# iden3/wasmsnark

Measured on AMD Instinct MI355X. Metric: BN128 Groth16 prove ms @ 2^20 constraints, lower is better.
Workload: dtype u256 (Montgomery; 9x29-bit limbs, v_mad_u64_u32); 1 GPU; BN128 full Groth16 prove, synthetic 2^20-constraint R1CS (1-3 non-zeros per column of A and B, every variable present), key and witness resident in HBM, r and s injected; parallelism=1 GPU, no collective, lanes=2, device=AMD Radeon Graphics gfx950:sramecc+:xnack- CUs=256 device=0

## Files before the change

wasmsnark_amd/csrc/msm.hip:

```cpp
#include <string.h>

#include <algorithm>
#include <chrono>

#include "internal.h"
namespace wsnark {

#ifndef WS_ACC_WAVES
#define WS_ACC_WAVES 3
#endif
#ifndef WS_ACC_WAVES_G2
#define WS_ACC_WAVES_G2 2
#endif
#ifndef WS_G2_PREFETCH
#define WS_G2_PREFETCH 0
#endif
#ifndef WS_G1_PREFETCH
#define WS_G1_PREFETCH 1
#endif
#ifndef WS_MADD_WIDE
#define WS_MADD_WIDE 1
#endif
static const uint32_t CHUNK = 8;
#ifndef WS_TAIL_L2_DEFAULT
#define WS_TAIL_L2_DEFAULT 4
#endif

struct MsmScratch {
    DevBuf vals_out, entries, hot, hot_sums;
    DevBuf bstart, bend, buckets, counters, tasks, multi, partials;
    DevBuf chunkS, chunkA, sums, points_conv;
    DevBuf hot_done;
    DevBuf tree_half, tree_done;
};

static const uint32_t PRESORT_MAX_BINS = 4096;
static const uint32_t CNT_HIST = 16, CNT_CURSOR = 16 + 512, CNT_BINS = 2048;

template <class Fn>
__device__ __forceinline__ void for_each_digit(const Fe& raw, uint32_t c, uint32_t Wall, uint32_t w_off, uint32_t w_stride, Fn f) {
    const Fe s = Fr::reduce_full(raw);
    const uint32_t NB = 1u << (c - 1);
    uint32_t carry = 0, k = 0;
    for (uint32_t w = 0; w < Wall; w++) {
        const uint32_t bit = w * c;
        const uint32_t limb = bit >> 6, off = bit & 63;
        uint64_t v = limb < 4 ? (s.l[limb] >> off) : 0;
        if (off + c > 64 && limb + 1 < 4) v |= s.l[limb + 1] << (64 - off);
        uint32_t d = (uint32_t)(v & ((1u << c) - 1)) + carry;
        uint32_t neg = 0;
        if (d > NB) { d = (1u << c) - d; neg = 1; carry = 1; } else carry = 0;
        if (w >= w_off && (w - w_off) % w_stride == 0) {
            if (d) f(k, d, neg);
            k++;
        }
    }
}

struct PresortArgs {
    const Fe* scalars;
    uint32_t n, c, Wall, w_off, w_stride;
    uint32_t i0, i_end;
    uint32_t lo_bits, HB, nbins;
    uint32_t tile;
    uint32_t idx_bits;
    const uint8_t* mask;
    uint32_t flat;
};
__device__ __forceinline__ uint32_t presort_bin(const PresortArgs& A, uint32_t k, uint32_t d) {
    return (A.flat ? 0u : k * A.HB) + ((d - 1) >> A.lo_bits);
}

template <class E> struct PresortEntry;
template <> struct PresortEntry<uint64_t> {
    static __device__ __forceinline__ uint64_t make(uint32_t i, uint32_t neg, uint32_t lo, uint32_t) {
        return ((uint64_t)lo << 32) | (uint64_t)(i | (neg << 31));
    }
    static __device__ __forceinline__ uint32_t lo(uint64_t e, uint32_t) { return (uint32_t)(e >> 32); }
    static __device__ __forceinline__ uint32_t val(uint64_t e, uint32_t) { return (uint32_t)e; }
};
template <> struct PresortEntry<uint32_t> {
    static __device__ __forceinline__ uint32_t make(uint32_t i, uint32_t neg, uint32_t lo, uint32_t ib) {
        return i | (neg << ib) | (lo << (ib + 1));
    }
    static __device__ __forceinline__ uint32_t lo(uint32_t e, uint32_t ib) { return e >> (ib + 1); }
    static __device__ __forceinline__ uint32_t val(uint32_t e, uint32_t ib) {
        return (e & ((1u << ib) - 1)) | (((e >> ib) & 1u) << 31);
    }
};

__global__ __launch_bounds__(1024) void presort_count(PresortArgs A, uint32_t* __restrict__ bin_count) {
    __shared__ uint32_t cnt[PRESORT_MAX_BINS];
    for (uint32_t b = threadIdx.x; b < A.nbins; b += blockDim.x) cnt[b] = 0;
    __syncthreads();
    const uint32_t base = A.i0 + blockIdx.x * A.tile;
    for (uint32_t i = base + threadIdx.x; i < base + A.tile && i < A.i_end; i += blockDim.x) {
        if (A.mask && !A.mask[i]) continue;
        for_each_digit(A.scalars[i], A.c, A.Wall, A.w_off, A.w_stride, [&](uint32_t k, uint32_t d, uint32_t) {
            atomicAdd(&cnt[presort_bin(A, k, d)], 1u);
        });
    }
    __syncthreads();
    for (uint32_t b = threadIdx.x; b < A.nbins; b += blockDim.x)
        if (cnt[b]) atomicAdd(&bin_count[b], cnt[b]);
}

__global__ __launch_bounds__(256) void presort_scan(const uint32_t* __restrict__ bin_count, uint32_t nbins,
                                                      uint32_t* __restrict__ bin_start, uint32_t* __restrict__ bin_cursor) {
    __shared__ uint32_t part[256];
    const uint32_t per = (nbins + 255) / 256, lo = threadIdx.x * per;
    uint32_t sum = 0;
    for (uint32_t b = lo; b < lo + per && b < nbins; b++) sum += bin_count[b];
    part[threadIdx.x] = sum;
    __syncthreads();
    if (threadIdx.x == 0) {
        uint32_t run = 0;
        for (uint32_t t = 0; t < 256; t++) { const uint32_t v = part[t]; part[t] = run; run += v; }
        bin_start[nbins] = run;
    }
    __syncthreads();
    uint32_t run = part[threadIdx.x];
    for (uint32_t b = lo; b < lo + per && b < nbins; b++) {
        bin_start[b] = run;
        bin_cursor[b] = run;
        run += bin_count[b];
    }
}

template <class E>
__global__ __launch_bounds__(1024) void presort_scatter(PresortArgs A, uint32_t* __restrict__ bin_cursor, E* __restrict__ entries) {
    __shared__ uint32_t cnt[PRESORT_MAX_BINS];
    __shared__ uint32_t gbase[PRESORT_MAX_BINS];
    for (uint32_t b = threadIdx.x; b < A.nbins; b += blockDim.x) cnt[b] = 0;
    __syncthreads();
    const uint32_t base = A.i0 + blockIdx.x * A.tile;
    for (uint32_t i = base + threadIdx.x; i < base + A.tile && i < A.i_end; i += blockDim.x) {
        if (A.mask && !A.mask[i]) continue;
        for_each_digit(A.scalars[i], A.c, A.Wall, A.w_off, A.w_stride, [&](uint32_t k, uint32_t d, uint32_t) {
            atomicAdd(&cnt[presort_bin(A, k, d)], 1u);
        });
    }
    __syncthreads();
    for (uint32_t b = threadIdx.x; b < A.nbins; b += blockDim.x) {
        const uint32_t c0 = cnt[b];
        gbase[b] = c0 ? atomicAdd(&bin_cursor[b], c0) : 0;
        cnt[b] = 0;
    }
    __syncthreads();
    const uint32_t lo_mask = (1u << A.lo_bits) - 1;
    for (uint32_t i = base + threadIdx.x; i < base + A.tile && i < A.i_end; i += blockDim.x) {
        if (A.mask && !A.mask[i]) continue;
        for_each_digit(A.scalars[i], A.c, A.Wall, A.w_off, A.w_stride, [&](uint32_t k, uint32_t d, uint32_t neg) {
            const uint32_t b = presort_bin(A, k, d);
            const uint32_t r = atomicAdd(&cnt[b], 1u);
            const uint32_t idx = A.flat ? (A.w_off + k * A.w_stride) * A.n + i : i;
            entries[gbase[b] + r] = PresortEntry<E>::make(idx, neg, (d - 1) & lo_mask, A.idx_bits);
        });
    }
}

static const uint32_t PRESORT_ONCE_W = 16;
__device__ __forceinline__ uint32_t block_exclusive_scan(uint32_t v, uint32_t* wsum, uint32_t* total) {
    const uint32_t lane = threadIdx.x & 63, wid = threadIdx.x >> 6, nw = (blockDim.x + 63) >> 6;
    uint32_t x = v;
    for (uint32_t d = 1; d < 64; d <<= 1) {
        const uint32_t y = __shfl(x, (int)(lane >= d ? lane - d : lane));
        if (lane >= d) x += y;
    }
    if (lane == 63) wsum[wid] = x;
    __syncthreads();
    if (wid == 0) {
        const uint32_t w = lane < nw ? wsum[lane] : 0;
        uint32_t t = w;
        for (uint32_t d = 1; d < 64; d <<= 1) {
            const uint32_t y = __shfl(t, (int)(lane >= d ? lane - d : lane));
            if (lane >= d) t += y;
        }
        if (lane < nw) wsum[lane] = t - w;
        if (lane == 63) wsum[16] = t;
    }
    __syncthreads();
    *total = wsum[16];
    return wsum[wid] + x - v;
}
template <class E>
__global__ __launch_bounds__(1024) void presort_scatter_once(PresortArgs A, const uint32_t* __restrict__ bin_count,
                                                               uint32_t* __restrict__ bin_start, uint32_t* __restrict__ bin_cursor,
                                                               E* __restrict__ entries) {
    __shared__ uint32_t cnt[PRESORT_MAX_BINS];
    __shared__ uint32_t gbase[PRESORT_MAX_BINS];
    __shared__ uint32_t wsum[17];
    {
        const uint32_t per = (A.nbins + blockDim.x - 1) / blockDim.x, b0 = threadIdx.x * per;
        uint32_t mine = 0, total;
        for (uint32_t b = b0; b < b0 + per && b < A.nbins; b++) mine += bin_count[b];
        uint32_t run = block_exclusive_scan(mine, wsum, &total);
        for (uint32_t b = b0; b < b0 + per && b < A.nbins; b++) {
            gbase[b] = run;
            if (blockIdx.x == 0) bin_start[b] = run;
            run += bin_count[b];
            cnt[b] = 0;
        }
        if (blockIdx.x == 0 && threadIdx.x == 0) bin_start[A.nbins] = total;
    }
    __syncthreads();
    const uint32_t i = A.i0 + blockIdx.x * blockDim.x + threadIdx.x;
    const bool live = i < A.i_end && (!A.mask || A.mask[i]);
    const uint32_t NONE = 0xFFFFFFFFu;
    E ent[PRESORT_ONCE_W];
    uint32_t where[PRESORT_ONCE_W];
    {
        const Fe s = live ? Fr::reduce_full(A.scalars[i]) : Fe{{0, 0, 0, 0}};
        const uint32_t c = A.c, NB = 1u << (c - 1), lo_mask = (1u << A.lo_bits) - 1;
        uint32_t carry = 0, k = 0, next_own = A.w_off;
#pragma unroll
        for (uint32_t w = 0; w < PRESORT_ONCE_W; w++) {
            where[w] = NONE;
            ent[w] = 0;
            if (w < A.Wall) {
                const uint32_t bit = w * c, limb = bit >> 6, off = bit & 63;
                const uint64_t lo = limb == 0 ? s.l[0] : limb == 1 ? s.l[1] : limb == 2 ? s.l[2] : limb == 3 ? s.l[3] : 0;
                const uint64_t hi = limb == 0 ? s.l[1] : limb == 1 ? s.l[2] : limb == 2 ? s.l[3] : 0;
                uint64_t v = lo >> off;
                if (off + c > 64) v |= hi << (64 - off);
                uint32_t d = (uint32_t)(v & ((1u << c) - 1)) + carry;
                uint32_t neg = 0;
                if (d > NB) { d = (1u << c) - d; neg = 1; carry = 1; } else carry = 0;
                if (w == next_own) {
                    if (live && d) {
                        const uint32_t b = presort_bin(A, k, d);
                        where[w] = b | (atomicAdd(&cnt[b], 1u) << 12);
                        ent[w] = PresortEntry<E>::make(A.flat ? w * A.n + i : i, neg, (d - 1) & lo_mask, A.idx_bits);
                    }
                    k++;
                    next_own += A.w_stride;
                }
            }
        }
    }
    __syncthreads();
    for (uint32_t b = threadIdx.x; b < A.nbins; b += blockDim.x) {
        const uint32_t c0 = cnt[b];
        if (c0) gbase[b] += atomicAdd(&bin_cursor[b], c0);
    }
    __syncthreads();
#pragma unroll
    for (uint32_t w = 0; w < PRESORT_ONCE_W; w++)
        if (where[w] != NONE) entries[gbase[where[w] & 0xFFFu] + (where[w] >> 12)] = ent[w];
}

__device__ __forceinline__ uint32_t len_key(uint32_t len, uint32_t lmax) {
    uint32_t k = (len * 255u + lmax - 1) / lmax;
    return k > 255u ? 255u : (k < 1u ? 1u : k);
}

static const uint32_t PRESORT_MAX_LO = 10;
__device__ __forceinline__ uint32_t wave_rank_add(uint32_t* counters, uint32_t key, bool active) {
    const unsigned long long act = __ballot(active);
    if (act == 0) return 0;
    const uint32_t lane = threadIdx.x & 63;
    const int first = __ffsll(act) - 1;
    const uint32_t k0 = __shfl(key, first);
    const unsigned long long same = __ballot(active && key == k0);
    uint32_t r = 0;
    if (same == act) {
        uint32_t base = 0;
        if (lane == (uint32_t)first) base = atomicAdd(&counters[k0], (uint32_t)__popcll(act));
        base = __shfl(base, first);
        r = base + (uint32_t)__popcll(act & ((1ull << lane) - 1));
    } else if (active) {
        r = atomicAdd(&counters[key], 1u);
    }
    return r;
}

template <class E>
__global__ __launch_bounds__(1024) void presort_bins(const E* __restrict__ entries, const uint32_t* __restrict__ bin_start,
                                                       uint32_t lo_bits, uint32_t idx_bits, uint32_t* __restrict__ vals_out,
                                                       uint32_t* __restrict__ bstart, uint32_t* __restrict__ bend,
                                                       uint32_t lmax, uint32_t* __restrict__ hist,
                                                       const uint8_t* __restrict__ mask, uint32_t mask_mod) {
    __shared__ uint32_t sub[1u << PRESORT_MAX_LO];
    __shared__ uint32_t off[1u << PRESORT_MAX_LO];
    __shared__ uint32_t wsum[17];
    __shared__ uint32_t lhist[256];
    const uint32_t bin = blockIdx.x, SUB = 1u << lo_bits;
    const uint32_t s = bin_start[bin], e = bin_start[bin + 1];
    for (uint32_t t = threadIdx.x; t < SUB; t += blockDim.x) sub[t] = 0;
    for (uint32_t t = threadIdx.x; t < 256; t += blockDim.x) lhist[t] = 0;
    __syncthreads();
    const uint32_t stride = 4 * blockDim.x;
    const uint32_t iters = (e - s + stride - 1) / stride;
    for (uint32_t it = 0; it < iters; it++) {
        const uint32_t i = s + threadIdx.x + it * stride;
        E v[4];
#pragma unroll
        for (uint32_t u = 0; u < 4; u++) {
            const uint32_t j = i + u * blockDim.x;
            v[u] = j < e ? entries[j] : (E)0;
        }
#pragma unroll
        for (uint32_t u = 0; u < 4; u++) {
            bool active = i + u * blockDim.x < e;
            if (mask && active) {
                const uint32_t idx = PresortEntry<E>::val(v[u], idx_bits) & 0x7FFFFFFFu;
                active = mask[mask_mod ? idx % mask_mod : idx] != 0;
            }
            (void)wave_rank_add(sub, PresortEntry<E>::lo(v[u], idx_bits), active);
        }
    }
    __syncthreads();
    const uint32_t per = (SUB + blockDim.x - 1) / blockDim.x, t0 = threadIdx.x * per;
    uint32_t mine = 0, bin_total;
    for (uint32_t t = t0; t < t0 + per && t < SUB; t++) mine += sub[t];
    uint32_t run = s + block_exclusive_scan(mine, wsum, &bin_total);
    for (uint32_t t = t0; t < t0 + per && t < SUB; t++) {
        const uint32_t cnt = sub[t];
        const uint32_t bucket = (bin << lo_bits) + t;
        off[t] = run;
        bstart[bucket] = run;
        bend[bucket] = run + cnt;
        run += cnt;
        sub[t] = 0;
        if (cnt) {
            const uint32_t nt = (cnt + lmax - 1) / lmax, rem = cnt - (nt - 1) * lmax;
            if (nt > 1) atomicAdd(&lhist[255], nt - 1);
            atomicAdd(&lhist[len_key(rem, lmax)], 1u);
        }
    }
    __syncthreads();
    for (uint32_t t = threadIdx.x; t < 256; t += blockDim.x)
        if (lhist[t]) atomicAdd(&hist[t], lhist[t]);
    for (uint32_t it = 0; it < iters; it++) {
        const uint32_t i = s + threadIdx.x + it * stride;
        E v[4];
#pragma unroll
        for (uint32_t u = 0; u < 4; u++) {
            const uint32_t j = i + u * blockDim.x;
            v[u] = j < e ? entries[j] : (E)0;
        }
#pragma unroll
        for (uint32_t u = 0; u < 4; u++) {
            bool active = i + u * blockDim.x < e;
            if (mask && active) {
                const uint32_t idx = PresortEntry<E>::val(v[u], idx_bits) & 0x7FFFFFFFu;
                active = mask[mask_mod ? idx % mask_mod : idx] != 0;
            }
            const uint32_t lo = PresortEntry<E>::lo(v[u], idx_bits);
            const uint32_t r = wave_rank_add(sub, lo, active);
            if (active) vals_out[off[lo] + r] = PresortEntry<E>::val(v[u], idx_bits);
        }
    }
}

#ifndef WS_ACC_FAST
#define WS_ACC_FAST 1
#endif
#ifndef WS_ACC_MMADD
#define WS_ACC_MMADD 1
#endif
template <class C>
__device__ __forceinline__ typename C::Pt accumulate_range(const typename C::AffP* __restrict__ points,
                                                           const uint32_t* __restrict__ vals, uint32_t s, uint32_t len) {
    typedef typename C::Field F;
    typename C::Pt acc = C::infinity();
    if (len == 0) return acc;
    constexpr bool kPrefetch = sizeof(typename C::AffP) > 64 ? WS_G2_PREFETCH != 0 : WS_G1_PREFETCH != 0;
    uint32_t k = 0;
#if WS_ACC_FAST && WS_MADD_WIDE
    {
        uint32_t v = vals[s];
        typename C::AffP cp = points[v & 0x7FFFFFFFu];
        if (!F::packed_is_zero(cp.x)) {
            typename C::Aff a0 = C::unpack_aff(cp);
            a0.y = F::cneg(a0.y, (v >> 31) != 0);
            acc = typename C::Pt{a0.x, a0.y, F::one(), F::one()};
            k = 1;
            const uint32_t last = len - 1;
#if WS_ACC_MMADD
            if (len > 1) {
                v = vals[s + 1];
                cp = points[v & 0x7FFFFFFFu];
                if (!F::packed_is_zero(cp.x) && C::mmadd_fast(acc, a0, C::unpack_aff(cp), (v >> 31) != 0)) k = 2;
            }
#endif
            if (kPrefetch) {
                uint32_t v1 = vals[s + (k < last ? k : last)], v2 = vals[s + (k + 1 < last ? k + 1 : last)];
                cp = points[v1 & 0x7FFFFFFFu];
                while (k < len) {
                    const bool inf = F::packed_is_zero(cp.x);
                    typename C::Aff cur = C::unpack_aff(cp);
                    const bool neg = (v1 >> 31) != 0;
                    F::keep(cur.x);
                    F::keep(cur.y);
                    v1 = v2;
                    cp = points[v1 & 0x7FFFFFFFu];
                    v2 = vals[s + (k + 2 < last ? k + 2 : last)];
                    if (inf) break;
                    if (!C::madd_fast(acc, cur, neg)) break;
                    k++;
                }
            } else {
                uint32_t vn = vals[s + (k < last ? k : last)];
                while (k < len) {
                    v = vn;
                    cp = points[v & 0x7FFFFFFFu];
                    vn = vals[s + (k + 1 < last ? k + 1 : last)];
                    if (F::packed_is_zero(cp.x)) break;
                    if (!C::madd_fast(acc, C::unpack_aff(cp), (v >> 31) != 0)) break;
                    k++;
                }
            }
        }
    }
#endif
    if (k < len) {
        if (!kPrefetch) {
            for (; k < len; k++) {
                const uint32_t v = vals[s + k];
                const typename C::Aff cur = C::unpack_aff(points[v & 0x7FFFFFFFu]);
#if WS_MADD_WIDE
                C::madd_wide(acc, cur, (v >> 31) != 0);
#else
                C::madd(acc, cur, (v >> 31) != 0);
#endif
            }
        } else {
            uint32_t v = vals[s + k];
            typename C::AffP nxt = points[v & 0x7FFFFFFFu];
            for (; k < len; k++) {
                const typename C::Aff cur = C::unpack_aff(nxt);
                const bool neg = (v >> 31) != 0;
                if (k + 1 < len) {
                    v = vals[s + k + 1];
                    nxt = points[v & 0x7FFFFFFFu];
                }
#if WS_MADD_WIDE
                C::madd_wide(acc, cur, neg);
#else
                C::madd(acc, cur, neg);
#endif
            }
        }
    }
    C::narrow_x(acc);
    return acc;
}

template <class C>
__global__ __launch_bounds__(256) void msm_convert_points(const typename C::AffP* __restrict__ in,
                                                            typename C::AffP* __restrict__ out, uint64_t n) {
    const uint64_t i = (uint64_t)blockIdx.x * blockDim.x + threadIdx.x;
    if (i >= n) return;
    out[i] = C::pack_aff(C::aff_to_internal(in[i]));
}

static const uint32_t PARTIAL_FLAG = 0x80000000u;
struct Task { uint32_t dst, start, len; };
struct MultiBucket { uint32_t bucket, first_partial, ntasks; };
static const uint32_t HOT_MIN = 1024;
static const uint32_t HOT_SLICE = 512;
struct HotBucket { uint32_t bucket, first_partial, ntasks, task_base, rem_index, start, rem, slice_base; };

__global__ __launch_bounds__(256) void msm_plan_emit(const uint32_t* __restrict__ bstart, const uint32_t* __restrict__ bend,
                                                       uint32_t nbuckets, uint32_t lmax, const uint32_t* __restrict__ hist,
                                                       uint32_t* __restrict__ cursor,
                                                       Task* __restrict__ tasks, uint32_t* __restrict__ counters,
                                                       MultiBucket* __restrict__ multi, HotBucket* __restrict__ hot,
                                                       uint32_t hot_min) {
    __shared__ uint32_t lcnt[256];
    __shared__ uint32_t lbase[256];
    __shared__ uint32_t first[256];
    lcnt[threadIdx.x] = 0;
    first[threadIdx.x] = hist[threadIdx.x];
    __syncthreads();
    for (uint32_t d = 1; d < 256; d <<= 1) {
        const uint32_t v = threadIdx.x + d < 256 ? first[threadIdx.x + d] : 0;
        __syncthreads();
        first[threadIdx.x] += v;
        __syncthreads();
    }
    if (blockIdx.x == 0 && threadIdx.x == 0) counters[3] = first[0];
    const uint32_t excl = threadIdx.x + 1 < 256 ? first[threadIdx.x + 1] : 0;
    __syncthreads();
    first[threadIdx.x] = excl;
// ... 483 lines not shown
        }
        for (uint32_t k = 0; k < logm; k++) acc = H::dbl(acc);
        for (uint32_t v = 0; v < I.tW; v++) acc = H::add(acc, sums[(size_t)v * I.nsum + I.logJ]);
        if (I.tW > 1) {
            HPt run = H::infinity(), tot = H::infinity();
            for (uint32_t v = I.tW - 1; v >= 1; v--) {
                run = H::add(run, sums[(size_t)v * I.nsum + I.logJ + 1]);
                tot = H::add(tot, run);
            }
            for (uint32_t k = 0; k < logt; k++) tot = H::dbl(tot);
            acc = H::add(acc, tot);
        }
        *out_host = acc;
        if (trace)
            fprintf(stderr, "[wsnark trace]   msm finish (%s, table): waited %.3f ms for the GPU, host tail %.3f ms\n", sizeof(HPt) > 128 ? "G2" : "G1",
                    std::chrono::duration<double, std::milli>(t_tail - t_wait).count(),
                    std::chrono::duration<double, std::milli>(std::chrono::steady_clock::now() - t_tail).count());
        return WS_OK;
    }
    uint32_t logm = 0, logt = 0, logP = 0;
    while ((1u << logm) < I.m) logm++;
    while ((1u << logt) < I.tNB) logt++;
    while ((1u << logP) < I.tP) logP++;
    const uint32_t rows_per_window = I.reduce ? I.nrows : I.nsum;
    HPt acc = H::infinity();
    bool started = false;
    for (int wg = (int)I.Wall - 1; wg >= 0; wg--) {
        const bool owned = (uint32_t)wg >= I.w_off && ((uint32_t)wg - I.w_off) % I.w_stride == 0;
        const uint32_t krow = owned ? ((uint32_t)wg - I.w_off) / I.w_stride : 0;
        const HPt* row = owned ? &sums[(size_t)krow * rows_per_window] : nullptr;
        for (int k = (int)I.c - 1; k >= 0; k--) {
            if (started) acc = H::dbl(acc);
            if (!owned) continue;
            if (I.reduce && (uint32_t)k >= logt && (uint32_t)k - logt < logP) { acc = H::add(acc, row[I.logJ + 1 + (uint32_t)k - logt]); started = true; }
            if ((uint32_t)k >= logm && (uint32_t)k - logm < I.logJ) { acc = H::add(acc, row[(uint32_t)k - logm]); started = true; }
            if (k == 0) { acc = H::add(acc, row[I.logJ]); started = true; }
        }
    }
    *out_host = acc;
    if (trace)
        fprintf(stderr, "[wsnark trace]   msm finish (%s): waited %.3f ms for the GPU, host Horner %.3f ms\n", sizeof(HPt) > 128 ? "G2" : "G1",
                std::chrono::duration<double, std::milli>(t_tail - t_wait).count(),
                std::chrono::duration<double, std::milli>(std::chrono::steady_clock::now() - t_tail).count());
    return WS_OK;
}

static int wait_plan_users(MsmWorkspace& M, int plan_id, hipStream_t s) {
    for (auto& p : M.slot)
        if (p.active && p.ev && p.info.n && p.plan_id == plan_id) WS_HIP_CHECK(hipStreamWaitEvent(s, p.ev, 0));
    return WS_OK;
}

uint32_t msm_table_rows(uint32_t tc) { return tc ? (255 + tc - 1) / tc : 1; }

uint32_t msm_table_window(uint64_t n) {
    { const long c = tuning_get("TABLE_C", 0); if (c >= 4 && c <= 22) return (uint32_t)c; }
    int lg = 0;
    while (((uint64_t)1 << (lg + 1)) <= n) lg++;
    int c = (n * 4 >= ((uint64_t)5 << lg)) ? lg + 1 : lg;
    if (c < 4) c = 4;
    if (c > 20) c = 20;
    return (uint32_t)c;
}

int msm_plan_begin(Lane& L, uint64_t n, WindowShard sh, hipStream_t s, uint32_t table_c) {
    Context* X = ctx();
    if (!X) return WS_ERR_NOINIT;
    if (!s) s = L.stream;
    MsmWorkspace& M = ws(L);
    MsmPlanInfo& I = M.plan[M.cur].info;
    I = MsmPlanInfo();
    if (n == 0) { I.valid = true; return WS_OK; }
    if (n > ((uint64_t)1 << 28)) return WS_ERR_SIZE;
    if (sh.stride == 0) return WS_ERR_ARG;
    I.n = n;
    I.flat = table_c != 0;
    I.c = I.flat ? table_c : pick_window(n);
    if (I.c < 2 || I.c > 22) return WS_ERR_ARG;
    I.Wall = (255 + I.c - 1) / I.c;
    if (I.flat && (uint64_t)I.Wall * n >= ((uint64_t)1 << 31)) return WS_ERR_SIZE;
    I.w_off = sh.off;
    I.w_stride = sh.stride;
    I.W = I.w_off < I.Wall ? (I.Wall - I.w_off + I.w_stride - 1) / I.w_stride : 0;
    if (I.W == 0) { I.n = 0; I.valid = true; return WS_OK; }
    I.NB = 1u << (I.c - 1);
    I.nbuckets = I.flat ? I.NB : I.W * I.NB;
    const uint64_t total = n * I.W;
    if (total >= ((uint64_t)1 << 32)) return WS_ERR_SIZE;
    const bool big_set = I.NB >= (1u << 18);
    uint32_t chunk = (I.flat && !big_set) ? 4u : CHUNK;
    { const long v = tuning_get("MSM_CHUNK", 0); if (v == 2 || v == 4 || v == 8 || v == 16 || v == 32) chunk = (uint32_t)v; }
    {
        uint32_t tbits = I.flat ? (big_set ? 15u : 11u) : 31u;
        { const long v = tuning_get("TAIL_BITS", 0); if (v >= 3 && v <= 20) tbits = (uint32_t)v; }
        I.tNB = (tbits >= 31 || I.NB < (1u << tbits)) ? I.NB : (1u << tbits);
        I.tP = I.NB / I.tNB;
        if (I.tP > 256) { I.tP = 256; I.tNB = I.NB / 256; }
        I.groups = I.flat ? 1 : I.W;
        I.tW = I.groups * I.tP;
    }
    I.m1 = I.tNB < chunk ? I.tNB : chunk;
    I.J1 = I.tNB / I.m1;
    I.m2 = 1;
    {
        long v = tuning_get("TAIL_L2", (I.flat && I.NB >= (1u << 17)) ? WS_TAIL_L2_DEFAULT : 1);
        if ((v == 2 || v == 4 || v == 8) && I.flat && I.tP > 1 && I.J1 >= 8u * (uint32_t)v) I.m2 = (uint32_t)v;
    }
    I.m = I.m1 * I.m2;
    I.J = I.J1 / I.m2;
    while ((1u << I.logJ) < I.J) I.logJ++;
    I.nsum = I.logJ + 1 + ((I.flat || I.tP > 1) ? 1 : 0) + (I.m2 > 1 ? 1 : 0);
    I.reduce = I.tP > 1;
    {
        uint32_t logP = 0;
        while ((1u << logP) < I.tP) logP++;
        I.nrows = I.reduce ? I.logJ + 1 + logP + (I.m2 > 1 ? 1 : 0) : I.nsum;
    }
    I.lmax = (uint32_t)(2 * (((I.flat ? total : n) + I.NB - 1) / I.NB));
    if (I.flat && I.NB < (1u << 19) && total >= ((uint64_t)1 << 22) && total / I.NB > 64) {
        const uint32_t by_tasks = (uint32_t)((total + (1u << 19) - 1) >> 19);
        if (I.lmax > by_tasks) I.lmax = by_tasks;
    }
    uint32_t lmin = 32;
    {
        if (I.nbuckets < (1u << 16) && total >= ((uint64_t)1 << 16)) {
            const uint32_t by_tasks = (uint32_t)((total + (1u << 17) - 1) >> 17);
            if (by_tasks < I.lmax) I.lmax = by_tasks;
            lmin = 8;
        } else if (I.flat && I.nbuckets == (1u << 16) && I.lmax > 16) {
            I.lmax = 16;
            lmin = 16;
        }
    }
    { const long v = tuning_get("MSM_LMAX", 0); if (v >= 4 && v <= 65536) { I.lmax = (uint32_t)v; lmin = 4; } }
    if (I.lmax < lmin) I.lmax = lmin;
    I.hot_cap = (uint32_t)(total / I.lmax) + I.nbuckets + 16;
    const uint32_t c = I.c, W = I.W, nbuckets = I.nbuckets, lmax = I.lmax;

    int rc = wait_plan_users(M, M.cur, s);
    if (rc) return rc;
    MsmScratch& S = M.plan[M.cur].S;
    WS_HIP_CHECK(S.vals_out.reserve(total * 4));
    WS_HIP_CHECK(S.bstart.reserve((size_t)nbuckets * 4));
    WS_HIP_CHECK(S.bend.reserve((size_t)nbuckets * 4));
    WS_HIP_CHECK(S.counters.reserve((size_t)CNT_BINS * 4 + ((size_t)PRESORT_MAX_BINS + 1) * 4 * 3));
    WS_HIP_CHECK(S.tasks.reserve((size_t)I.hot_cap * sizeof(Task)));
    WS_HIP_CHECK(S.multi.reserve((size_t)I.hot_cap * sizeof(MultiBucket)));
    uint32_t hot_min = HOT_MIN;
    { const long v = tuning_get("MSM_HOT_MIN", 0); if (v >= 2) hot_min = (uint32_t)v; }
    I.hot_min = hot_min;
    WS_HIP_CHECK(S.hot.reserve(((size_t)I.hot_cap / hot_min + 16) * sizeof(HotBucket)));

    uint32_t* d_cnt = S.counters.as<uint32_t>();
    const uint32_t env_lo = 8, env_tile = 1024, env_thr = 1024;
    const bool env_e64 = tuning_get("MSM_ENTRY64", 0) != 0;
    uint32_t lo_bits = env_lo > PRESORT_MAX_LO ? PRESORT_MAX_LO : env_lo;
    if (lo_bits > c - 1) lo_bits = c - 1;
    const uint32_t Wb = I.flat ? 1 : W;
    while ((uint64_t)Wb * (I.NB >> lo_bits) > PRESORT_MAX_BINS && lo_bits < c - 1 && lo_bits < PRESORT_MAX_LO) lo_bits++;
    while (I.flat && (I.NB >> lo_bits) < 2048 && lo_bits > 7) lo_bits--;
    uint32_t idx_bits = 1;
    while (((uint64_t)1 << idx_bits) < (I.flat ? (uint64_t)I.Wall * n : n)) idx_bits++;
    while (!env_e64 && idx_bits + 1 + lo_bits > 32 && lo_bits > 1 && (uint64_t)Wb * (I.NB >> (lo_bits - 1)) <= PRESORT_MAX_BINS) lo_bits--;
    const uint32_t HB = I.NB >> lo_bits, nbins = Wb * HB;
    if (nbins > PRESORT_MAX_BINS) { set_last_error("msm: grouping pass geometry out of range"); return WS_ERR_SIZE; }
    {
        const bool e32 = !env_e64 && idx_bits + 1 + lo_bits <= 32;
        WS_HIP_CHECK(S.entries.reserve(total * (e32 ? 4 : 8)));
        WS_HIP_CHECK(hipMemsetAsync(S.counters.p, 0, (CNT_BINS + 3 * ((size_t)nbins + 1)) * 4, s));
        I.ps_valid = true;
        I.ps_lo_bits = lo_bits; I.ps_idx_bits = idx_bits; I.ps_nbins = nbins; I.ps_e32 = e32;
        I.ps_HB = HB; I.ps_tile = env_tile; I.ps_thr = env_thr;
    }
    (void)d_cnt; (void)hot_min; (void)lmax; (void)nbuckets;
    I.building = true;
    return WS_OK;
}

static PresortArgs plan_presort_args(const MsmPlanInfo& I, const Fe* d_scalars, uint32_t i0, uint32_t i_end) {
    return PresortArgs{d_scalars, (uint32_t)I.n, I.c, I.Wall, I.w_off, I.w_stride, i0, i_end, I.ps_lo_bits, I.ps_HB, I.ps_nbins, I.ps_tile,
                       I.ps_idx_bits, nullptr, I.flat ? 1u : 0u};
}

int msm_plan_count(Lane& L, const Fe* d_scalars, uint64_t i0, uint64_t i1, hipStream_t s) {
    Context* X = ctx();
    if (!X) return WS_ERR_NOINIT;
    if (!s) s = L.stream;
    MsmWorkspace& M = ws(L);
    MsmPlanInfo& I = M.plan[M.cur].info;
    if (I.n == 0 && I.valid) return WS_OK;
    if (!I.building) { set_last_error("msm_plan_count: no plan is being built"); return WS_ERR_ARG; }
    if (!d_scalars || i0 > i1 || i1 > I.n) return WS_ERR_ARG;
    if (!I.ps_valid || i0 == i1) return WS_OK;
    MsmScratch& S = M.plan[M.cur].S;
    uint32_t* bin_count = S.counters.as<uint32_t>() + CNT_BINS;
    const PresortArgs PA = plan_presort_args(I, d_scalars, (uint32_t)i0, (uint32_t)i1);
    X->timer.begin("msm_presort_count", s);
    hipLaunchKernelGGL(presort_count, dim3(ceil_div_u64(i1 - i0, I.ps_tile)), dim3(I.ps_thr), 0, s, PA, bin_count);
    X->timer.end(s);
    WS_HIP_CHECK(hipGetLastError());
    return WS_OK;
}

int msm_plan_finish(Lane& L, const Fe* d_scalars, hipStream_t s) {
    Context* X = ctx();
    if (!X) return WS_ERR_NOINIT;
    if (!s) s = L.stream;
    MsmWorkspace& M = ws(L);
    MsmPlanInfo& I = M.plan[M.cur].info;
    if (I.n == 0 && I.valid) return WS_OK;
    if (!I.building) { set_last_error("msm_plan_finish: no plan is being built"); return WS_ERR_ARG; }
    if (!d_scalars) return WS_ERR_ARG;
    I.building = false;
    MsmScratch& S = M.plan[M.cur].S;
    KernelTimer& T = X->timer;
    const uint64_t n = I.n, total = n * I.W;
    const uint32_t nbuckets = I.nbuckets, lmax = I.lmax, hot_min = I.hot_min;
    uint32_t* d_cnt = S.counters.as<uint32_t>();
    if (I.ps_valid) {
        const uint32_t nbins = I.ps_nbins, lo_bits = I.ps_lo_bits, idx_bits = I.ps_idx_bits;
        const bool e32 = I.ps_e32;
        uint32_t* bin_count = d_cnt + CNT_BINS;
        uint32_t* bin_start = bin_count + (nbins + 1);
        uint32_t* bin_cursor = bin_start + (nbins + 1);
        const PresortArgs PA = plan_presort_args(I, d_scalars, 0u, (uint32_t)n);
        const dim3 grid(ceil_div_u64(n, I.ps_tile)), blk(I.ps_thr);
        const bool once = I.Wall <= PRESORT_ONCE_W && I.ps_tile == I.ps_thr;
        if (!once) {
            T.begin("msm_presort_scan", s);
            hipLaunchKernelGGL(presort_scan, dim3(1), dim3(256), 0, s, bin_count, nbins, bin_start, bin_cursor);
            T.end(s);
        }
        T.begin("msm_presort_scatter", s);
        if (once && e32) hipLaunchKernelGGL(presort_scatter_once<uint32_t>, grid, blk, 0, s, PA, bin_count, bin_start, bin_cursor, S.entries.as<uint32_t>());
        else if (once) hipLaunchKernelGGL(presort_scatter_once<uint64_t>, grid, blk, 0, s, PA, bin_count, bin_start, bin_cursor, S.entries.as<uint64_t>());
        else if (e32) hipLaunchKernelGGL(presort_scatter<uint32_t>, grid, blk, 0, s, PA, bin_cursor, S.entries.as<uint32_t>());
        else hipLaunchKernelGGL(presort_scatter<uint64_t>, grid, blk, 0, s, PA, bin_cursor, S.entries.as<uint64_t>());
        T.end(s);
        uint32_t bthr = (uint32_t)((total / nbins / 8 + 63) / 64 * 64);
        bthr = bthr < 64 ? 64 : bthr > 1024 ? 1024 : bthr;
        const dim3 bblk(bthr);
        T.begin("msm_presort_bins", s);
        if (e32)
            hipLaunchKernelGGL(presort_bins<uint32_t>, dim3(nbins), bblk, 0, s, S.entries.as<uint32_t>(), bin_start, lo_bits,
                               idx_bits, S.vals_out.as<uint32_t>(), S.bstart.as<uint32_t>(), S.bend.as<uint32_t>(), lmax, d_cnt + CNT_HIST, nullptr, 0u);
        else
            hipLaunchKernelGGL(presort_bins<uint64_t>, dim3(nbins), bblk, 0, s, S.entries.as<uint64_t>(), bin_start, lo_bits,
                               idx_bits, S.vals_out.as<uint32_t>(), S.bstart.as<uint32_t>(), S.bend.as<uint32_t>(), lmax, d_cnt + CNT_HIST, nullptr, 0u);
        T.end(s);
        WS_HIP_CHECK(hipGetLastError());
        I.ps_bthr = bthr;
    } else {
        set_last_error("msm_plan_finish: the plan has no grouping pass");
        return WS_ERR_ARG;
    }
    T.begin("msm_plan", s);
    hipLaunchKernelGGL(msm_plan_emit, dim3(ceil_div_u64(nbuckets, 256)), dim3(256), 0, s, S.bstart.as<uint32_t>(),
                       S.bend.as<uint32_t>(), nbuckets, lmax, d_cnt + CNT_HIST, d_cnt + CNT_CURSOR, S.tasks.as<Task>(), d_cnt,
                       S.multi.as<MultiBucket>(), S.hot.as<HotBucket>(), hot_min);
    hipLaunchKernelGGL(msm_plan_emit_hot, dim3(64), dim3(256), 0, s, S.hot.as<HotBucket>(), d_cnt, lmax, S.tasks.as<Task>());
    T.end(s);
    WS_HIP_CHECK(hipGetLastError());
    I.ntasks = I.hot_cap;
    I.nmulti = 0;
    I.valid = true;
    return WS_OK;
}


int msm_plan_dev(Lane& L, const Fe* d_scalars, uint64_t n, WindowShard sh, hipStream_t s, uint32_t table_c) {
    if (n && !d_scalars) return WS_ERR_ARG;
    int rc = msm_plan_begin(L, n, sh, s, table_c);
    if (!rc) rc = msm_plan_count(L, d_scalars, 0, n, s);
    if (!rc) rc = msm_plan_finish(L, d_scalars, s);
    return rc;
}

int msm_plan_variant(Lane& L, int src_id, int dst_id, const uint8_t* d_mask, hipStream_t s) {
    Context* X = ctx();
    if (!X) return WS_ERR_NOINIT;
    if (!s) s = L.stream;
    if (src_id < 0 || src_id >= kPlans || dst_id < 0 || dst_id >= kPlans || src_id == dst_id || !d_mask) return WS_ERR_ARG;
    MsmWorkspace& M = ws(L);
    const MsmPlanInfo src = M.plan[src_id].info;
    MsmScratch& SS = M.plan[src_id].S;
    MsmPlanInfo& I = M.plan[dst_id].info;
    MsmScratch& S = M.plan[dst_id].S;
    if (!src.valid || !src.ps_valid || src.n == 0) { set_last_error("msm_plan_variant: the source plan has no shared grouping pass"); return WS_ERR_ARG; }
    int rc = wait_plan_users(M, dst_id, s);
    if (rc) return rc;
    I = src;
    I.ps_valid = false;
    I.valid = false;
    const uint64_t total = src.n * src.W;
    WS_HIP_CHECK(S.vals_out.reserve(total * 4));
    WS_HIP_CHECK(S.bstart.reserve((size_t)src.nbuckets * 4));
    WS_HIP_CHECK(S.bend.reserve((size_t)src.nbuckets * 4));
    WS_HIP_CHECK(S.counters.reserve((size_t)CNT_BINS * 4 + ((size_t)PRESORT_MAX_BINS + 1) * 4 * 3));
    WS_HIP_CHECK(S.tasks.reserve((size_t)src.hot_cap * sizeof(Task)));
    WS_HIP_CHECK(S.multi.reserve((size_t)src.hot_cap * sizeof(MultiBucket)));
    WS_HIP_CHECK(S.hot.reserve(((size_t)src.hot_cap / src.hot_min + 16) * sizeof(HotBucket)));
    uint32_t* d_cnt = S.counters.as<uint32_t>();
    WS_HIP_CHECK(hipMemsetAsync(S.counters.p, 0, (size_t)CNT_BINS * 4, s));
    const uint32_t* bin_start = SS.counters.as<uint32_t>() + CNT_BINS + (src.ps_nbins + 1);
    KernelTimer& T = X->timer;
    T.begin("msm_presort_bins", s);
    if (src.ps_e32)
        hipLaunchKernelGGL(presort_bins<uint32_t>, dim3(src.ps_nbins), dim3(src.ps_bthr), 0, s, SS.entries.as<uint32_t>(), bin_start,
                           src.ps_lo_bits, src.ps_idx_bits, S.vals_out.as<uint32_t>(), S.bstart.as<uint32_t>(), S.bend.as<uint32_t>(),
                           src.lmax, d_cnt + CNT_HIST, d_mask, src.flat ? (uint32_t)src.n : 0u);
    else
        hipLaunchKernelGGL(presort_bins<uint64_t>, dim3(src.ps_nbins), dim3(src.ps_bthr), 0, s, SS.entries.as<uint64_t>(), bin_start,
                           src.ps_lo_bits, src.ps_idx_bits, S.vals_out.as<uint32_t>(), S.bstart.as<uint32_t>(), S.bend.as<uint32_t>(),
                           src.lmax, d_cnt + CNT_HIST, d_mask, src.flat ? (uint32_t)src.n : 0u);
    T.end(s);
    T.begin("msm_plan", s);
    hipLaunchKernelGGL(msm_plan_emit, dim3(ceil_div_u64(src.nbuckets, 256)), dim3(256), 0, s, S.bstart.as<uint32_t>(),
                       S.bend.as<uint32_t>(), src.nbuckets, src.lmax, d_cnt + CNT_HIST, d_cnt + CNT_CURSOR, S.tasks.as<Task>(), d_cnt,
                       S.multi.as<MultiBucket>(), S.hot.as<HotBucket>(), src.hot_min);
    hipLaunchKernelGGL(msm_plan_emit_hot, dim3(64), dim3(256), 0, s, S.hot.as<HotBucket>(), d_cnt, src.lmax, S.tasks.as<Task>());
    T.end(s);
    WS_HIP_CHECK(hipGetLastError());
    I.valid = true;
    return WS_OK;
}

template <class C>
static int msm_acc_sets(Lane& L, MsmPending* const* Ps, int nsets, int which, hipStream_t s) {
    typedef typename C::PtP Pt;
    Context* X = ctx();
    MsmWorkspace& M = ws(L);
    KernelTimer& T = X->timer;
    AccSets<C> as;
    uint32_t ntasks = 0, cb_small = CB_SMALL_MIN;
    for (int k = 0; k < 4; k++) {
        MsmPending& Q = *Ps[k < nsets ? k : 0];
        MsmScratch& QS = M.plan[Q.plan_id].S;
        as.points[k] = reinterpret_cast<const typename C::AffP*>(Q.d_points_used);
        as.vals[k] = QS.vals_out.as<uint32_t>();
        as.tasks[k] = QS.tasks.as<Task>();
        as.counters[k] = QS.counters.as<uint32_t>();
        as.multi[k] = QS.multi.as<MultiBucket>();
        as.hot[k] = QS.hot.as<HotBucket>();
        as.buckets[k] = Q.S.buckets.template as<Pt>();
        as.partials[k] = Q.S.partials.template as<Pt>();
        as.hot_sums[k] = Q.S.hot_sums.template as<Pt>();
        as.hot_done[k] = Q.S.hot_done.template as<uint32_t>();
        if (k < nsets && Q.info.ntasks > ntasks) ntasks = Q.info.ntasks;
        if (k < nsets) {
            const MsmPlanInfo& QI = Q.info;
            const uint64_t mean = (QI.n * QI.W + QI.nbuckets - 1) / (QI.nbuckets ? QI.nbuckets : 1);
            if (2 * (uint64_t)QI.lmax < 3 * mean) {
                const uint32_t want = (QI.nbuckets + 63) / 64;
                if (want > cb_small) cb_small = want > CB_SMALL_MAX ? CB_SMALL_MAX : want;
            }
        }
    }
    const uint32_t ny = (uint32_t)nsets;
    T.begin(which ? "msm_accumulate_g2" : "msm_accumulate_g1", s);
    hipLaunchKernelGGL(msm_accumulate<C>, dim3(ceil_div_u64(ntasks, 256), ny), dim3(256), 0, s, as);
    T.end(s);
    WS_HIP_CHECK(hipGetLastError());
    T.begin("msm_combine", s);
    hipLaunchKernelGGL(msm_combine_all<C>, dim3(cb_small + CB_WAVE + CB_HOT, ny), dim3(64), 0, s, as, cb_small);
    T.end(s);
    WS_HIP_CHECK(hipGetLastError());
    return WS_OK;
}

template <class C, class H>
static int msm_launch_acc(Lane& L, int which, const typename H::Aff* d_points_ref, bool prepared, int* slot_out, hipStream_t s, bool defer_kernels = false) {
    typedef typename C::PtP Pt;
    static_assert(sizeof(typename C::PtP) == sizeof(typename H::Pt) && sizeof(typename C::AffP) == sizeof(typename H::Aff), "layouts");
    Context* X = ctx();
    if (!X) return WS_ERR_NOINIT;
    if (!s) s = L.stream;
    MsmWorkspace& M = ws(L);
    const MsmPlanInfo& I = M.plan[M.cur].info;
    if (!I.valid) { set_last_error("msm: no plan"); return WS_ERR_ARG; }
    if (I.n && !d_points_ref) return WS_ERR_ARG;
    int slot = -1;
    for (int i = 0; i < kPendingSlots; i++) if (!M.slot[i].active) { slot = i; break; }
    if (slot < 0) { set_last_error("msm: too many unfinished launches"); return WS_ERR_ARG; }
    MsmPending& P = M.slot[slot];
    P.which = which;
    P.info = I;
    P.plan_id = M.cur;
    P.partner = -1;
    if (I.n == 0) { P.active = true; *slot_out = slot; return WS_OK; }
    const typename C::AffP* d_points = reinterpret_cast<const typename C::AffP*>(d_points_ref);
    const uint64_t n = I.n;
    const uint32_t W = I.tW, nbuckets = I.nbuckets, J = I.J, nsum = I.nsum;

    MsmScratch& S = P.S;
    WS_HIP_CHECK(S.buckets.reserve((size_t)nbuckets * sizeof(Pt)));
    WS_HIP_CHECK(S.partials.reserve((size_t)I.hot_cap * sizeof(Pt)));
    WS_HIP_CHECK(S.chunkS.reserve(((size_t)W * I.J1 + (I.m2 > 1 ? (size_t)2 * W * J : 0)) * sizeof(Pt)));
    WS_HIP_CHECK(S.chunkA.reserve(((size_t)W * I.J1 + (I.m2 > 1 ? (size_t)W * J : 0)) * sizeof(Pt)));
    const size_t sums_bytes = (I.reduce ? (size_t)I.groups * I.nrows : (size_t)W * nsum) * sizeof(Pt);
    WS_HIP_CHECK(P.d_sums.reserve(sums_bytes));
    if (I.reduce) WS_HIP_CHECK(P.d_rows.reserve((size_t)W * nsum * sizeof(Pt)));
    WS_HIP_CHECK(S.tree_half.reserve((size_t)W * 6 * sizeof(Pt)));
    {
        const size_t db = (size_t)W * 3 * sizeof(uint32_t);
        if (!S.tree_done.p || S.tree_done.bytes < db) { WS_HIP_CHECK(S.tree_done.alloc(db)); WS_HIP_CHECK(hipMemsetAsync(S.tree_done.p, 0, db, s)); }
    }
    if (P.h_bytes < sums_bytes) {
        if (P.h_sums) (void)hipHostFree(P.h_sums);
        P.h_sums = nullptr; P.h_bytes = 0;
        WS_HIP_CHECK(hipHostMalloc(&P.h_sums, sums_bytes, 0));
        P.h_bytes = sums_bytes;
    }
    if (!P.ev) WS_HIP_CHECK(hipEventCreate(&P.ev));
    WS_HIP_CHECK(S.hot_sums.reserve(((size_t)I.hot_cap / HOT_SLICE + (size_t)I.hot_cap / I.hot_min + 32) * sizeof(Pt)));
    {
        const size_t hot_bytes = ((size_t)I.hot_cap / I.hot_min + 16) * 4;
        if (!S.hot_done.p || S.hot_done.bytes < hot_bytes) { WS_HIP_CHECK(S.hot_done.alloc(hot_bytes)); WS_HIP_CHECK(hipMemsetAsync(S.hot_done.p, 0, hot_bytes, s)); }
    }

    KernelTimer& T = X->timer;
    if (I.flat && !prepared) { set_last_error("msm: a table plan needs a prepared fixed-base table"); return WS_ERR_ARG; }
    if (C::Field::kInternalDomain && !prepared) {
        WS_HIP_CHECK(S.points_conv.reserve((size_t)n * sizeof(typename C::AffP)));
        T.begin("msm_convert_points", s);
        hipLaunchKernelGGL(msm_convert_points<C>, dim3(ceil_div_u64(n, 256)), dim3(256), 0, s, d_points,
                           S.points_conv.as<typename C::AffP>(), n);
        T.end(s);
        d_points = S.points_conv.as<typename C::AffP>();
    }
    P.d_points_used = d_points;
    if (!defer_kernels) {
        MsmPending* one[1] = {&P};
        int rc = msm_acc_sets<C>(L, one, 1, which, s);
        if (rc) return rc;
    }
    P.active = true;
    *slot_out = slot;
    return WS_OK;
}

template <class C> struct TailCurve { typedef C type; typedef C paired; };
template <> struct TailCurve<G1R29> { typedef G1R29I type; typedef G1P29 paired; };
template <> struct TailCurve<G2R29> { typedef G2P29 type; typedef G2Q29 paired; };
static bool tail_pair_g1() { return tuning_get("TAIL_PAIR_G1", 1) != 0; }
static bool tail_quad_g2() { return tuning_get("TAIL_QUAD_G2", 1) != 0; }
template <class C> static bool tail_split() { return sizeof(typename C::AffP) > 64 ? tail_quad_g2() : tail_pair_g1(); }
template <class C, class CC = C>
static int msm_launch_tail(Lane& L, const int* slot_ids, int nslots, hipStream_t s, int second_slot = -1) {
    typedef PointIO<C> IO;
    typedef typename IO::Stored St;
    static_assert(sizeof(typename PointIO<CC>::Stored) == sizeof(St), "the chunk and tree kernels share their buffers");
    Context* X = ctx();
    if (!s) s = L.stream;
    MsmPending* slots = ws(L).slot;
    const MsmPlanInfo& I = slots[slot_ids[0]].info;
    if (I.n == 0) return WS_OK;
    TailSets<C> ts;
    for (int k = 0; k < 4; k++) {
        MsmPending& P = slots[slot_ids[k < nslots ? k : 0]];
        ts.buckets[k] = P.S.buckets.template as<St>();
        ts.l1S[k] = P.S.chunkS.template as<St>();
        ts.l1A[k] = P.S.chunkA.template as<St>();
        ts.chunkS[k] = P.S.chunkS.template as<St>() + (I.m2 > 1 ? (size_t)I.tW * I.J1 : 0);
        ts.chunkA[k] = P.S.chunkA.template as<St>() + (I.m2 > 1 ? (size_t)I.tW * I.J1 : 0);
        ts.chunkW[k] = P.S.chunkS.template as<St>() + (size_t)I.tW * I.J1 + (size_t)I.tW * I.J;
        ts.rows[k] = P.d_rows.template as<St>();
        ts.sums[k] = P.d_sums.template as<St>();
// ... 461 lines not shown
```

Before: 8.522 ms.

## Stage presort scatter and bin outputs in LDS for coalesced global writes

```diff
diff --git a/wasmsnark_amd/csrc/msm.hip b/wasmsnark_amd/csrc/msm.hip
--- a/wasmsnark_amd/csrc/msm.hip
+++ b/wasmsnark_amd/csrc/msm.hip
@@ -160,6 +160,11 @@
 }
 
 static const uint32_t PRESORT_ONCE_W = 16;
+static const uint32_t PRESORT_LDS_BYTES = 160u << 10;
+constexpr uint32_t presort_stage_lds(uint32_t rows) { return 2 * PRESORT_MAX_BINS * 4 + rows * 1024 * (4 + 2) + 17 * 4; }
+constexpr bool presort_stage_fits(uint32_t rows) { return rows == 0 || (presort_stage_lds(rows) <= PRESORT_LDS_BYTES && presort_stage_fits(rows - 1)); }
+static_assert(presort_stage_fits(PRESORT_ONCE_W), "the staged scatter's LDS exceeds a CU's for some row count up to PRESORT_ONCE_W");
+static_assert(PRESORT_MAX_BINS <= 1u << 12 && PRESORT_ONCE_W * 1024 <= 1u << 20, "where[]: 12 bits of bin, 20 of rank");
 __device__ __forceinline__ uint32_t block_exclusive_scan(uint32_t v, uint32_t* wsum, uint32_t* total) {
     const uint32_t lane = threadIdx.x & 63, wid = threadIdx.x >> 6, nw = (blockDim.x + 63) >> 6;
     uint32_t x = v;
@@ -183,7 +188,7 @@
     *total = wsum[16];
     return wsum[wid] + x - v;
 }
-template <class E>
+template <class E, bool STAGED>
 __global__ __launch_bounds__(1024) void presort_scatter_once(PresortArgs A, const uint32_t* __restrict__ bin_count,
                                                                uint32_t* __restrict__ bin_start, uint32_t* __restrict__ bin_cursor,
                                                                E* __restrict__ entries) {
@@ -239,14 +244,40 @@
         }
     }
     __syncthreads();
-    for (uint32_t b = threadIdx.x; b < A.nbins; b += blockDim.x) {
-        const uint32_t c0 = cnt[b];
-        if (c0) gbase[b] += atomicAdd(&bin_cursor[b], c0);
-    }
-    __syncthreads();
+    if constexpr (STAGED) {
+        static_assert(sizeof(E) == 4, "the stage holds 4-byte entries");
+        __shared__ uint32_t stage[PRESORT_ONCE_W * 1024];
+        __shared__ uint16_t stage_bin[PRESORT_ONCE_W * 1024];
+        const uint32_t per = (A.nbins + blockDim.x - 1) / blockDim.x, b0 = threadIdx.x * per;
+        uint32_t mine = 0, staged;
+        for (uint32_t b = b0; b < b0 + per && b < A.nbins; b++) mine += cnt[b];
+        uint32_t run = block_exclusive_scan(mine, wsum, &staged);
+        for (uint32_t b = b0; b < b0 + per && b < A.nbins; b++) {
+            const uint32_t c0 = cnt[b];
+            if (c0) gbase[b] += atomicAdd(&bin_cursor[b], c0) - run;
+            cnt[b] = run;
+            run += c0;
+        }
+        __syncthreads();
 #pragma unroll
-    for (uint32_t w = 0; w < PRESORT_ONCE_W; w++)
-        if (where[w] != NONE) entries[gbase[where[w] & 0xFFFu] + (where[w] >> 12)] = ent[w];
+        for (uint32_t w = 0; w < PRESORT_ONCE_W; w++)
+            if (where[w] != NONE) {
+                const uint32_t b = where[w] & 0xFFFu, j = cnt[b] + (where[w] >> 12);
+                stage[j] = ent[w];
+                stage_bin[j] = (uint16_t)b;
+            }
+        __syncthreads();
+        for (uint32_t j = threadIdx.x; j < staged; j += blockDim.x) entries[gbase[stage_bin[j]] + j] = stage[j];
+    } else {
+        for (uint32_t b = threadIdx.x; b < A.nbins; b += blockDim.x) {
+            const uint32_t c0 = cnt[b];
+            if (c0) gbase[b] += atomicAdd(&bin_cursor[b], c0);
+        }
+        __syncthreads();
+#pragma unroll
+        for (uint32_t w = 0; w < PRESORT_ONCE_W; w++)
+            if (where[w] != NONE) entries[gbase[where[w] & 0xFFFu] + (where[w] >> 12)] = ent[w];
+    }
 }
 
 __device__ __forceinline__ uint32_t len_key(uint32_t len, uint32_t lmax) {
@@ -274,42 +305,10 @@
     return r;
 }
 
-template <class E>
-__global__ __launch_bounds__(1024) void presort_bins(const E* __restrict__ entries, const uint32_t* __restrict__ bin_start,
-                                                       uint32_t lo_bits, uint32_t idx_bits, uint32_t* __restrict__ vals_out,
-                                                       uint32_t* __restrict__ bstart, uint32_t* __restrict__ bend,
-                                                       uint32_t lmax, uint32_t* __restrict__ hist,
-                                                       const uint8_t* __restrict__ mask, uint32_t mask_mod) {
-    __shared__ uint32_t sub[1u << PRESORT_MAX_LO];
-    __shared__ uint32_t off[1u << PRESORT_MAX_LO];
-    __shared__ uint32_t wsum[17];
-    __shared__ uint32_t lhist[256];
-    const uint32_t bin = blockIdx.x, SUB = 1u << lo_bits;
-    const uint32_t s = bin_start[bin], e = bin_start[bin + 1];
-    for (uint32_t t = threadIdx.x; t < SUB; t += blockDim.x) sub[t] = 0;
-    for (uint32_t t = threadIdx.x; t < 256; t += blockDim.x) lhist[t] = 0;
-    __syncthreads();
-    const uint32_t stride = 4 * blockDim.x;
-    const uint32_t iters = (e - s + stride - 1) / stride;
-    for (uint32_t it = 0; it < iters; it++) {
-        const uint32_t i = s + threadIdx.x + it * stride;
-        E v[4];
-#pragma unroll
-        for (uint32_t u = 0; u < 4; u++) {
-            const uint32_t j = i + u * blockDim.x;
-            v[u] = j < e ? entries[j] : (E)0;
-        }
-#pragma unroll
-        for (uint32_t u = 0; u < 4; u++) {
-            bool active = i + u * blockDim.x < e;
-            if (mask && active) {
-                const uint32_t idx = PresortEntry<E>::val(v[u], idx_bits) & 0x7FFFFFFFu;
-                active = mask[mask_mod ? idx % mask_mod : idx] != 0;
-            }
-            (void)wave_rank_add(sub, PresortEntry<E>::lo(v[u], idx_bits), active);
-        }
-    }
-    __syncthreads();
+__device__ __forceinline__ uint32_t presort_bins_bounds(uint32_t bin, uint32_t s, uint32_t lo_bits, uint32_t lmax, uint32_t* sub, uint32_t* off,
+                                                        uint32_t* wsum, uint32_t* lhist, uint32_t* __restrict__ bstart,
+                                                        uint32_t* __restrict__ bend, uint32_t* __restrict__ hist) {
+    const uint32_t SUB = 1u << lo_bits;
     const uint32_t per = (SUB + blockDim.x - 1) / blockDim.x, t0 = threadIdx.x * per;
     uint32_t mine = 0, bin_total;
     for (uint32_t t = t0; t < t0 + per && t < SUB; t++) mine += sub[t];
@@ -331,6 +330,93 @@
     __syncthreads();
     for (uint32_t t = threadIdx.x; t < 256; t += blockDim.x)
         if (lhist[t]) atomicAdd(&hist[t], lhist[t]);
+    return bin_total;
+}
+
+static const uint32_t PRESORT_BINS_CAP = 4096;
+static_assert(PRESORT_BINS_CAP < 0xFFFFu, "ranks are kept in 16 bits, 0xFFFF marks a masked entry");
+static_assert(PRESORT_BINS_CAP * (4 + 4 + 2) + (2u << PRESORT_MAX_LO) * 4 + (17 + 256) * 4 <= PRESORT_LDS_BYTES / 3, "staged presort_bins: three workgroups per CU");
+template <class E, bool STAGED>
+__global__ __launch_bounds__(1024) void presort_bins(const E* __restrict__ entries, const uint32_t* __restrict__ bin_start,
+                                                       uint32_t lo_bits, uint32_t idx_bits, uint32_t* __restrict__ vals_out,
+                                                       uint32_t* __restrict__ bstart, uint32_t* __restrict__ bend,
+                                                       uint32_t lmax, uint32_t* __restrict__ hist,
+                                                       const uint8_t* __restrict__ mask, uint32_t mask_mod) {
+    __shared__ uint32_t sub[1u << PRESORT_MAX_LO];
+    __shared__ uint32_t off[1u << PRESORT_MAX_LO];
+    __shared__ uint32_t wsum[17];
+    __shared__ uint32_t lhist[256];
+    const uint32_t bin = blockIdx.x, SUB = 1u << lo_bits;
+    const uint32_t s = bin_start[bin], e = bin_start[bin + 1];
+    for (uint32_t t = threadIdx.x; t < SUB; t += blockDim.x) sub[t] = 0;
+    for (uint32_t t = threadIdx.x; t < 256; t += blockDim.x) lhist[t] = 0;
+    __syncthreads();
+    const uint32_t stride = 4 * blockDim.x;
+    const uint32_t iters = (e - s + stride - 1) / stride;
+    const bool staged = STAGED && e - s <= PRESORT_BINS_CAP;
+    (void)staged;
+    if constexpr (STAGED) {
+        __shared__ uint32_t st_in[PRESORT_BINS_CAP];
+        __shared__ uint32_t st_out[PRESORT_BINS_CAP];
+        __shared__ uint16_t st_rank[PRESORT_BINS_CAP];
+        if (staged) {
+            for (uint32_t it = 0; it < iters; it++) {
+                const uint32_t i = s + threadIdx.x + it * stride;
+                E v[4];
+#pragma unroll
+                for (uint32_t u = 0; u < 4; u++) {
+                    const uint32_t j = i + u * blockDim.x;
+                    v[u] = j < e ? entries[j] : (E)0;
+                }
+#pragma unroll
+                for (uint32_t u = 0; u < 4; u++) {
+                    const uint32_t j = i + u * blockDim.x;
+                    bool active = j < e;
+                    if (mask && active) {
+                        const uint32_t idx = PresortEntry<E>::val(v[u], idx_bits) & 0x7FFFFFFFu;
+                        active = mask[mask_mod ? idx % mask_mod : idx] != 0;
+                    }
+                    const uint32_t r = wave_rank_add(sub, PresortEntry<E>::lo(v[u], idx_bits), active);
+                    if (j < e) {
+                        st_in[j - s] = (uint32_t)v[u];
+                        st_rank[j - s] = active ? (uint16_t)r : (uint16_t)0xFFFFu;
+                    }
+                }
+            }
+            __syncthreads();
+            const uint32_t kept = presort_bins_bounds(bin, s, lo_bits, lmax, sub, off, wsum, lhist, bstart, bend, hist);
+            for (uint32_t j = threadIdx.x; j < e - s; j += blockDim.x) {
+                const uint32_t r = st_rank[j];
+                if (r != 0xFFFFu) {
+                    const E v = (E)st_in[j];
+                    st_out[off[PresortEntry<E>::lo(v, idx_bits)] - s + r] = PresortEntry<E>::val(v, idx_bits);
+                }
+            }
+            __syncthreads();
+            for (uint32_t j = threadIdx.x; j < kept; j += blockDim.x) vals_out[s + j] = st_out[j];
+            return;
+        }
+    }
+    for (uint32_t it = 0; it < iters; it++) {
+        const uint32_t i = s + threadIdx.x + it * stride;
+        E v[4];
+#pragma unroll
+        for (uint32_t u = 0; u < 4; u++) {
+            const uint32_t j = i + u * blockDim.x;
+            v[u] = j < e ? entries[j] : (E)0;
+        }
+#pragma unroll
+        for (uint32_t u = 0; u < 4; u++) {
+            bool active = i + u * blockDim.x < e;
+            if (mask && active) {
+                const uint32_t idx = PresortEntry<E>::val(v[u], idx_bits) & 0x7FFFFFFFu;
+                active = mask[mask_mod ? idx % mask_mod : idx] != 0;
+            }
+            (void)wave_rank_add(sub, PresortEntry<E>::lo(v[u], idx_bits), active);
+        }
+    }
+    __syncthreads();
+    (void)presort_bins_bounds(bin, s, lo_bits, lmax, sub, off, wsum, lhist, bstart, bend, hist);
     for (uint32_t it = 0; it < iters; it++) {
         const uint32_t i = s + threadIdx.x + it * stride;
         E v[4];
@@ -1120,7 +1206,9 @@
     WS_HIP_CHECK(S.hot.reserve(((size_t)I.hot_cap / hot_min + 16) * sizeof(HotBucket)));
 
     uint32_t* d_cnt = S.counters.as<uint32_t>();
-    const uint32_t env_lo = 8, env_tile = 1024, env_thr = 1024;
+    uint32_t env_lo = 8;
+    const uint32_t env_tile = 1024, env_thr = 1024;
+    { const long v = tuning_get("MSM_LO_BITS", 0); if (v >= 1 && v <= (long)PRESORT_MAX_LO) env_lo = (uint32_t)v; }
     const bool env_e64 = tuning_get("MSM_ENTRY64", 0) != 0;
     uint32_t lo_bits = env_lo > PRESORT_MAX_LO ? PRESORT_MAX_LO : env_lo;
     if (lo_bits > c - 1) lo_bits = c - 1;
@@ -1145,6 +1233,26 @@
     return WS_OK;
 }
 
+static bool presort_stage_scatter() { const long v = tuning_get("PRESORT_STAGE", 1); return v == 1 || v == 2; }
+static bool presort_stage_bins() { const long v = tuning_get("PRESORT_STAGE", 1); return v == 1 || v == 3; }
+
+static void launch_presort_bins(const MsmPlanInfo& I, uint32_t bthr, const MsmScratch& src, const uint32_t* bin_start, MsmScratch& S, uint32_t* hist,
+                                const uint8_t* mask, uint32_t mask_mod, hipStream_t s) {
+    const dim3 grid(I.ps_nbins), blk(bthr);
+    uint32_t* vals = S.vals_out.as<uint32_t>();
+    uint32_t* bs = S.bstart.as<uint32_t>();
+    uint32_t* be = S.bend.as<uint32_t>();
+    if (I.ps_e32 && presort_stage_bins())
+        hipLaunchKernelGGL((presort_bins<uint32_t, true>), grid, blk, 0, s, src.entries.as<uint32_t>(), bin_start, I.ps_lo_bits, I.ps_idx_bits, vals, bs, be,
+                           I.lmax, hist, mask, mask_mod);
+    else if (I.ps_e32)
+        hipLaunchKernelGGL((presort_bins<uint32_t, false>), grid, blk, 0, s, src.entries.as<uint32_t>(), bin_start, I.ps_lo_bits, I.ps_idx_bits, vals, bs, be,
+                           I.lmax, hist, mask, mask_mod);
+    else
+        hipLaunchKernelGGL((presort_bins<uint64_t, false>), grid, blk, 0, s, src.entries.as<uint64_t>(), bin_start, I.ps_lo_bits, I.ps_idx_bits, vals, bs, be,
+                           I.lmax, hist, mask, mask_mod);
+}
+
 static PresortArgs plan_presort_args(const MsmPlanInfo& I, const Fe* d_scalars, uint32_t i0, uint32_t i_end) {
     return PresortArgs{d_scalars, (uint32_t)I.n, I.c, I.Wall, I.w_off, I.w_stride, i0, i_end, I.ps_lo_bits, I.ps_HB, I.ps_nbins, I.ps_tile,
                        I.ps_idx_bits, nullptr, I.flat ? 1u : 0u};
@@ -1186,7 +1294,7 @@
     const uint32_t nbuckets = I.nbuckets, lmax = I.lmax, hot_min = I.hot_min;
     uint32_t* d_cnt = S.counters.as<uint32_t>();
     if (I.ps_valid) {
-        const uint32_t nbins = I.ps_nbins, lo_bits = I.ps_lo_bits, idx_bits = I.ps_idx_bits;
+        const uint32_t nbins = I.ps_nbins;
         const bool e32 = I.ps_e32;
         uint32_t* bin_count = d_cnt + CNT_BINS;
         uint32_t* bin_start = bin_count + (nbins + 1);
@@ -1200,21 +1308,17 @@
             T.end(s);
         }
         T.begin("msm_presort_scatter", s);
-        if (once && e32) hipLaunchKernelGGL(presort_scatter_once<uint32_t>, grid, blk, 0, s, PA, bin_count, bin_start, bin_cursor, S.entries.as<uint32_t>());
-        else if (once) hipLaunchKernelGGL(presort_scatter_once<uint64_t>, grid, blk, 0, s, PA, bin_count, bin_start, bin_cursor, S.entries.as<uint64_t>());
+        if (once && e32 && presort_stage_scatter())
+            hipLaunchKernelGGL((presort_scatter_once<uint32_t, true>), grid, blk, 0, s, PA, bin_count, bin_start, bin_cursor, S.entries.as<uint32_t>());
+        else if (once && e32) hipLaunchKernelGGL((presort_scatter_once<uint32_t, false>), grid, blk, 0, s, PA, bin_count, bin_start, bin_cursor, S.entries.as<uint32_t>());
+        else if (once) hipLaunchKernelGGL((presort_scatter_once<uint64_t, false>), grid, blk, 0, s, PA, bin_count, bin_start, bin_cursor, S.entries.as<uint64_t>());
         else if (e32) hipLaunchKernelGGL(presort_scatter<uint32_t>, grid, blk, 0, s, PA, bin_cursor, S.entries.as<uint32_t>());
         else hipLaunchKernelGGL(presort_scatter<uint64_t>, grid, blk, 0, s, PA, bin_cursor, S.entries.as<uint64_t>());
         T.end(s);
         uint32_t bthr = (uint32_t)((total / nbins / 8 + 63) / 64 * 64);
         bthr = bthr < 64 ? 64 : bthr > 1024 ? 1024 : bthr;
-        const dim3 bblk(bthr);
         T.begin("msm_presort_bins", s);
-        if (e32)
-            hipLaunchKernelGGL(presort_bins<uint32_t>, dim3(nbins), bblk, 0, s, S.entries.as<uint32_t>(), bin_start, lo_bits,
-                               idx_bits, S.vals_out.as<uint32_t>(), S.bstart.as<uint32_t>(), S.bend.as<uint32_t>(), lmax, d_cnt + CNT_HIST, nullptr, 0u);
-        else
-            hipLaunchKernelGGL(presort_bins<uint64_t>, dim3(nbins), bblk, 0, s, S.entries.as<uint64_t>(), bin_start, lo_bits,
-                               idx_bits, S.vals_out.as<uint32_t>(), S.bstart.as<uint32_t>(), S.bend.as<uint32_t>(), lmax, d_cnt + CNT_HIST, nullptr, 0u);
+        launch_presort_bins(I, bthr, S, bin_start, S, d_cnt + CNT_HIST, nullptr, 0u, s);
         T.end(s);
         WS_HIP_CHECK(hipGetLastError());
         I.ps_bthr = bthr;
@@ -1273,14 +1377,7 @@
     const uint32_t* bin_start = SS.counters.as<uint32_t>() + CNT_BINS + (src.ps_nbins + 1);
     KernelTimer& T = X->timer;
     T.begin("msm_presort_bins", s);
-    if (src.ps_e32)
-        hipLaunchKernelGGL(presort_bins<uint32_t>, dim3(src.ps_nbins), dim3(src.ps_bthr), 0, s, SS.entries.as<uint32_t>(), bin_start,
-                           src.ps_lo_bits, src.ps_idx_bits, S.vals_out.as<uint32_t>(), S.bstart.as<uint32_t>(), S.bend.as<uint32_t>(),
-                           src.lmax, d_cnt + CNT_HIST, d_mask, src.flat ? (uint32_t)src.n : 0u);
-    else
-        hipLaunchKernelGGL(presort_bins<uint64_t>, dim3(src.ps_nbins), dim3(src.ps_bthr), 0, s, SS.entries.as<uint64_t>(), bin_start,
-                           src.ps_lo_bits, src.ps_idx_bits, S.vals_out.as<uint32_t>(), S.bstart.as<uint32_t>(), S.bend.as<uint32_t>(),
-                           src.lmax, d_cnt + CNT_HIST, d_mask, src.flat ? (uint32_t)src.n : 0u);
+    launch_presort_bins(src, src.ps_bthr, SS, bin_start, S, d_cnt + CNT_HIST, d_mask, src.flat ? (uint32_t)src.n : 0u, s);
     T.end(s);
     T.begin("msm_plan", s);
     hipLaunchKernelGGL(msm_plan_emit, dim3(ceil_div_u64(src.nbuckets, 256)), dim3(256), 0, s, S.bstart.as<uint32_t>(),
```

Result: faster. 8.412 ms, median of 6 (-1.3%).
